# ChuhanZhou/News_Recommendation_Model

Hardware: NVIDIA B200
Metric: train_impressions_per_sec (higher is better)
Workload: dtype f32 (pair products as 3 x bf16 tcgen05 MMAs, fp32 accumulate; meets the fp32 tolerances)

## Files before the change

news_recommendation_model_b200/csrc/nrm_api.cu:

```cuda
#include <cstdarg>
#include <cstdio>
#include <cstring>
#include <mutex>
#include <vector>

#include "nrm_kernels.cuh"

namespace nrm {

static thread_local char g_err[512] = "";

void set_error(const char* fmt, ...) {
  va_list ap;
  va_start(ap, fmt);
  vsnprintf(g_err, sizeof(g_err), fmt, ap);
  va_end(ap);
}
int cuda_fail(cudaError_t e, const char* what) {
  set_error("CUDA error %d (%s) at %s", (int)e, cudaGetErrorString(e), what);
  return NRM_ECUDA;
}
int current_device() {
  int dev = 0;
  if (cudaGetDevice(&dev) != cudaSuccess || dev < 0 || dev >= 64) return 0;
// ... 22 lines not shown

KernelTimer::KernelTimer(const char* name, cudaStream_t stream) : slot_(-1), stream_(stream) {
  if (!g_timing) return;
  std::lock_guard<std::mutex> lock(g_timer_mu);
  int s = -1;
  for (int i = 0; i < g_ntimers; ++i) if (strcmp(g_timers[i].name, name) == 0) { s = i; break; }
  if (s < 0) { if (g_ntimers == kTimerSlots) return; s = g_ntimers++; g_timers[s].name = name; g_timers[s].used = 0; g_timers[s].made = false; }
  TimerSlot& t = g_timers[s];
  if (!t.made) { for (int i = 0; i < kTimerRing; ++i) { cudaEventCreate(&t.beg[i]); cudaEventCreate(&t.end[i]); } t.made = true; }
  if (t.used >= kTimerRing) return;
  slot_ = s;
  cudaEventRecord(t.beg[t.used], stream_);
}
KernelTimer::~KernelTimer() {
  if (slot_ < 0) return;
  std::lock_guard<std::mutex> lock(g_timer_mu);
  TimerSlot& t = g_timers[slot_];
  cudaEventRecord(t.end[t.used], stream_);
  t.used++;
}

struct SideStream {
  int dev; cudaStream_t caller;
  cudaStream_t stream; cudaEvent_t fork, join, fork2, join2, fork0, join0, join_tp, fork3, join3, fork4, join4;
  bool head_wgrad_pending = false; const float* wg_params = nullptr; float* wg_grads = nullptr; int wg_tiles = 0, wg_precision = 0;
};
static std::mutex g_side_mu;
static std::vector<SideStream*> g_sides;
static SideStream* side_stream(cudaStream_t caller) {
  const int dev = current_device();
  std::lock_guard<std::mutex> lock(g_side_mu);
  for (SideStream* p : g_sides)
    if (p->dev == dev && p->caller == caller) return p;
  SideStream* ss = new SideStream();
  ss->dev = dev; ss->caller = caller;
  bool ok = cudaStreamCreateWithFlags(&ss->stream, cudaStreamNonBlocking) == cudaSuccess;
  cudaEvent_t* evs[] = {&ss->fork, &ss->join, &ss->fork2, &ss->join2, &ss->fork0, &ss->join0, &ss->join_tp, &ss->fork3, &ss->join3,
                        &ss->fork4, &ss->join4};
  for (cudaEvent_t* e : evs) ok = ok && cudaEventCreateWithFlags(e, cudaEventDisableTiming) == cudaSuccess;
  if (!ok) { delete ss; return nullptr; }
  g_sides.push_back(ss);
  return ss;
}

bool use_rowstacked() {
  static const bool on = getenv("NRM_ATT_ITEM_TILES") == nullptr;
  return on;
}

bool w1_forward_on_tensor_cores(const Workspace&) {
  static const bool on = getenv("NRM_W1_FWD_TC") != nullptr;
  return on;
}

bool pdl_enabled() {
  static const bool on = getenv("NRM_NO_PDL") == nullptr;
  return on;
}

struct LayoutEntry { const char* name; long long offset; long long numel; };
// ... 44 lines not shown
  w.B = B; w.H = H; w.C = C;
  w.NH = (long long)B * H; w.R = (long long)B * C; w.N = w.NH + w.R;
  size_t off = 0;
  auto take = [&](size_t bytes) -> void* {
    void* p = base ? (char*)base + off : nullptr;
    off += (bytes + 255) & ~(size_t)255;
    return p;
  };
  const size_t f = sizeof(float);
  const size_t NH = (size_t)w.NH, R = (size_t)w.R, N = (size_t)w.N;
  w.xin_h = (float*)take(f * NH * XIN);
  w.xh = (float*)take(f * NH * 64);
  w.pca_h = (float*)take(f * NH * 64);
  w.e = (float*)take(f * R * E);
  w.mean = (float*)take(f * E);
  w.rstd = (float*)take(f * E);
  w.bn_sums = (double*)take(sizeof(double) * 2 * E);
  w.stat_part = (double*)take(sizeof(double) * STAT_BLOCKS * 2 * E);
  w.a1 = (float*)take(f * R * HID);
  w.gate = (float*)take(f * R * E);
  w.a2 = (float*)take(f * R * HID);
  w.y = (float*)take(f * R * E);
  w.a3 = (float*)take(f * R * HID);
  w.head_wt = (float*)take(f * (HEAD_WT_W1T + 64 * XIN));
  w.att_derived = (float*)take(f * 2 * 12420);
  w.tp = (float*)take(f * 2 * R * 64);
  w.att_rs_img = (float*)take(attention_rs_image_bytes());
  w.head_img = (float*)take(head_tc_image_bytes());
  w.head_arrive = (unsigned int*)take(256);
  if (training) {
    w.da3 = (float*)take(f * R * HID); w.da2 = (float*)take(f * R * HID); w.da1 = (float*)take(f * R * HID);
    w.dy = (float*)take(f * R * E);
    w.dgate = (float*)take(f * R * E);
    w.de = (float*)take(f * R * E);
    w.dz = (float*)take(f * R * E);
    w.bn_bwd_sums = (double*)take(sizeof(double) * 2 * E);
    w.head_part_f = (float*)take(f * ((R + 31) / 32) * 68);
    w.head_part_bn = (double*)take(sizeof(double) * ((R + 31) / 32) * 2 * E);
    w.head_part_w = (float*)take(f * 5 * HEAD_WG_CHUNKS_MAX * (HID * E + E));
    w.dxh = (float*)take(f * NH * 64);
    w.dxt = (float*)take(f * R * 64);
    w.dxin_h = (float*)take(f * NH * XIN);
    {
      const size_t ffma = (size_t)ATT_BWD_CTAS_MAX * ATT_PARTIAL, tc = (size_t)ATT_TC_PARTS_MAX * ATT_TC_PARTIAL;
      w.att_part = (float*)take(f * 2 * (ffma > tc ? ffma : tc));
    }
    w.dtp = (float*)take(f * 2 * R * 64);
// ... 29 lines not shown
  if (B <= 0 || H <= 0 || C <= 0) { set_error("%s: B, H, C must be positive (got %d, %d, %d)", fn, B, H, C); return NRM_EINVAL; }
  if (((long long)B * H + (long long)B * C) * 6 >= (1LL << 31)) { set_error("%s: batch too large for 32-bit entry ids", fn); return NRM_EINVAL; }
  return NRM_OK;
}
static int get_workspace(const char* fn, Workspace& w, void* ws, size_t ws_bytes, int B, int H, int C, int mode) {
  if (ws == nullptr || ((uintptr_t)ws & 255) != 0) { set_error("%s: workspace must be non-null and 256-byte aligned", fn); return NRM_EWORKSPACE; }
  const size_t need = carve_workspace(w, ws, B, H, C, mode);
  if (need > ws_bytes) { set_error("%s: workspace too small (%zu < %zu bytes)", fn, ws_bytes, need); return NRM_EWORKSPACE; }
  return NRM_OK;
}

static int encoder_forward(const BatchPtrs& in, const float* P, Workspace& w, int mode, int precision, cudaStream_t s) {
  SideStream* ss = side_stream(s);
  if (ss == nullptr) { set_error("encoder_forward: cannot create the side stream"); return NRM_ECUDA; }
  const bool tc = precision != NRM_PRECISION_FP32;
  NRM_CUDA(cudaEventRecord(ss->fork0, s));
  NRM_CUDA(cudaStreamWaitEvent(ss->stream, ss->fork0, 0));
  NRM_TRY(launch_head_transpose(P, w, ss->stream));
  NRM_CUDA(cudaEventRecord(ss->join0, ss->stream));
  if (tc) {
    if (use_rowstacked()) NRM_TRY(launch_attention_prep_rs(P, w, ss->stream)); else NRM_TRY(launch_attention_prep(P, w, ss->stream));
    if (head_on_tensor_cores(precision)) NRM_TRY(launch_head_images_tc(P, w, precision, (mode & NRM_MODE_KEEP_FOR_BWD) != 0, ss->stream));
  }
  { KernelTimer t("embed_rows", s);
    NRM_TRY(launch_embed_rows(in, P, w, (mode & NRM_MODE_KEEP_FOR_BWD) != 0, s)); }
  NRM_CUDA(cudaEventRecord(ss->fork, s));
  NRM_CUDA(cudaStreamWaitEvent(ss->stream, ss->fork, 0));
  if (tc) NRM_TRY(launch_candidate_tp(P, w, ss->stream));
  NRM_CUDA(cudaEventRecord(ss->join_tp, ss->stream));
  if (mode & NRM_MODE_KEEP_FOR_BWD) {
    NRM_TRY(launch_table_sort(w, ss->stream));
    NRM_CUDA(cudaEventRecord(ss->join, ss->stream));
  }
  NRM_CUDA(cudaStreamWaitEvent(s, ss->join0, 0));
  { KernelTimer t("w1_forward", s);
    if (tc && use_rowstacked() && w1_forward_on_tensor_cores(w)) NRM_TRY(launch_w1_forward_tc(P, w, precision, s)); else NRM_TRY(launch_w1_forward(P, w, s)); }
  NRM_CUDA(cudaStreamWaitEvent(s, ss->join_tp, 0));
  if (!tc) {
    { KernelTimer t("attention_forward_label", s); NRM_TRY(launch_attention_forward(in, P, w, 0, precision, s)); }
    { KernelTimer t("attention_forward_textimg", s); NRM_TRY(launch_attention_forward(in, P, w, 1, precision, s)); }
  } else {
    KernelTimer t("attention_forward", s);
    if (use_rowstacked()) {
      NRM_TRY(launch_attention_forward_rs(in, w, precision, s));
    } else {
      NRM_TRY(launch_attention_forward(in, P, w, 0, precision, s));
      NRM_TRY(launch_attention_forward(in, P, w, 1, precision, s));
    }
  }
  if (mode & NRM_MODE_KEEP_FOR_BWD) NRM_CUDA(cudaStreamWaitEvent(s, ss->join, 0));
  return NRM_OK;
}

static int encoder_backward(const BatchPtrs& in, const float* P, Workspace& w, int precision, float* G, cudaStream_t s) {
  SideStream* ss = side_stream(s);
  if (ss == nullptr) { set_error("encoder_backward: cannot create the side stream"); return NRM_ECUDA; }
  { KernelTimer t("attention_backward_label", s); NRM_TRY(launch_attention_backward(in, P, w, 0, precision, s)); }
  if (precision != NRM_PRECISION_FP32 && use_rowstacked()) {
    KernelTimer t("attention_input_grad_label", s);
    NRM_TRY(launch_attention_input_grad_rs(w, precision, s));
// ... 47 lines not shown
      NRM_CUDA(cudaEventSynchronize(t.end[k]));
      NRM_CUDA(cudaEventElapsedTime(&ms, t.beg[k], t.end[k]));
      total += ms;
    }
    float t_beg = 0.f, t_end = 0.f;
    if (t.used > 0 && g_ntimers > 0 && g_timers[0].used > 0) {
      cudaEventElapsedTime(&t_beg, g_timers[0].beg[g_timers[0].used - 1], t.beg[t.used - 1]);
      cudaEventElapsedTime(&t_end, g_timers[0].beg[g_timers[0].used - 1], t.end[t.used - 1]);
    }
    const int n = snprintf(buf + off, buf_bytes - off, "%s %d %.6f %.6f %.6f\n", t.name, t.used, total, t_beg, t_end);
    if (n < 0 || (size_t)n >= buf_bytes - off) break;
    off += (size_t)n;
  }
  return NRM_OK;
}
extern "C" int nrm_debug_rsprof(long long* host_out64) { return rsprof_read(host_out64); }
extern "C" long long nrm_debug_ws_field(int B, int H, int C, int mode, const char* name, long long* bytes) {
  if (B <= 0 || H <= 0 || C <= 0 || !name || !bytes) return -1;
  Workspace w;
  carve_workspace(w, reinterpret_cast<void*>(uintptr_t(256)), B, H, C, mode);
  const size_t R = (size_t)w.R, NH = (size_t)w.NH;
  struct F { const char* n; const void* p; size_t b; };
  const F fields[] = {{"e", w.e, R * E * 4}, {"de", w.de, R * E * 4}, {"dz", w.dz, R * E * 4}, {"dxh", w.dxh, NH * 64 * 4}, {"dxt", w.dxt, R * 64 * 4},
                      {"dxin_h", w.dxin_h, NH * XIN * 4}, {"att_dhid", w.att_dhid, (size_t)attention_rs_tiles(B, H, C) * 2 * 16384},
                      {"att_sc", w.att_sc, (size_t)attention_rs_tiles(B, H, C) * 512 * 4}, {"xh", w.xh, NH * 64 * 4}, {"dtp", w.dtp, 2 * R * 64 * 4},
                      {"tp", w.tp, 2 * R * 64 * 4}};
  for (const F& f : fields)
    if (strcmp(f.n, name) == 0 && f.p != nullptr) { *bytes = (long long)f.b; return (long long)(reinterpret_cast<uintptr_t>(f.p) - 256); }
  return -1;
}
extern "C" int nrm_debug_headprof(long long* host_out32) { return headprof_read(host_out32); }
extern "C" const char* nrm_last_error(void) { return g_err; }
extern "C" int nrm_layout_entries(void) { return kLayoutEntries; }
extern "C" const char* nrm_layout_name(int i) { return (i >= 0 && i < kLayoutEntries) ? kLayout[i].name : nullptr; }
extern "C" long long nrm_layout_offset(int i) { return (i >= 0 && i < kLayoutEntries) ? kLayout[i].offset : -1; }
extern "C" long long nrm_layout_numel(int i) { return (i >= 0 && i < kLayoutEntries) ? kLayout[i].numel : -1; }
extern "C" long long nrm_layout_fixed_floats(void) { return P_DELTA; }

extern "C" size_t nrm_workspace_bytes(int B, int H, int C, int mode) {
  if (B <= 0 || H <= 0 || C <= 0) return 0;
  Workspace w;
  return carve_workspace(w, nullptr, B, H, C, mode);
}

extern "C" size_t nrm_workspace_e_offset(int B, int H, int C, int mode) {
  if (B <= 0 || H <= 0 || C <= 0) return 0;
  Workspace w;
// ... 314 lines not shown
```

news_recommendation_model_b200/csrc/nrm_attention_tc.cu:

```cuda
#include "nrm_kernels.cuh"
#include <cstddef>

#include "nrm_umma.cuh"

namespace nrm {

#ifdef NRM_TC_PROFILE
__device__ long long g_tcprof[32];
#define TCPROF_DECL long long tcp_t = clock64();
#define TCPROF(i) do { if (blockIdx.x == 0 && (threadIdx.x == 0 || threadIdx.x == 32)) { const long long n__ = clock64(); g_tcprof[(i) + (threadIdx.x ? 16 : 0)] += n__ - tcp_t; tcp_t = n__; } } while (0)
#else
#define TCPROF_DECL
#define TCPROF(i) do { } while (0)
#endif

constexpr int TC_THREADS = 256;
constexpr int TC_MAXC = 8;

constexpr int DER_WD = 0, DER_A = 4096, DER_W2 = 8192, DER_B2 = 8256, DER_SIZE = 12420;
__host__ __device__ constexpr int wda_index(int j, int k) { return (((k >> 3) * 2 + ((k >> 2) & 1)) * 64 + j) * 4 + (k & 3); }

__global__ void __launch_bounds__(256)
att_prep_kernel(const float* __restrict__ P, float* __restrict__ der) {
  pdl_wait();
  pdl_trigger();
  const AttOffsets off = blockIdx.y == 0 ? ATT_LABEL : ATT_TI;
  float* d = der + (long long)blockIdx.y * DER_SIZE;
  const float* W = P + off.fc1_w;
  for (int i = blockIdx.x * 256 + threadIdx.x; i < 4096; i += gridDim.x * 256) {
    const int j = i >> 6, k = i & 63;
    const float wa = W[j * 256 + k], wc = W[j * 256 + 128 + k], wd = W[j * 256 + 192 + k];
    d[DER_WD + wda_index(j, k)] = wd;
    d[DER_A + wda_index(j, k)] = wa - wc;
  }
  if (blockIdx.x == 0 && threadIdx.x < 64) {
    d[DER_W2 + threadIdx.x] = P[off.fc2_w + threadIdx.x];
    if (threadIdx.x == 0) d[DER_B2] = P[off.fc2_b];
  }
}

__global__ void __launch_bounds__(256)
candidate_tp_kernel(const float* __restrict__ P, const float* __restrict__ e, long long R, float* __restrict__ tp_all) {
  pdl_wait();
  pdl_trigger();
  __shared__ float st[32][65];
  __shared__ float sBT[64][65];
  const AttOffsets off = blockIdx.y == 0 ? ATT_LABEL : ATT_TI;
  const int toff = blockIdx.y == 0 ? E_XT : E_PCAT;
  const float* W = P + off.fc1_w;
  float* tp = tp_all + (long long)blockIdx.y * R * 64;
  const int tid = threadIdx.x;
  const long long r0 = (long long)blockIdx.x * 32;
  const int nr = (int)min(32LL, R - r0);
  for (int i = tid; i < 32 * 64; i += 256) {
    const int r = i >> 6, k = i & 63;
    st[r][k] = r < nr ? __ldg(e + (r0 + r) * E + toff + k) : 0.f;
  }
  for (int i = tid; i < 64 * 64; i += 256) {
    const int j = i >> 6, k = i & 63;
    sBT[k][j] = __ldg(W + j * 256 + 64 + k) + __ldg(W + j * 256 + 128 + k);
  }
  __syncthreads();
  const int r = tid >> 3, jq = tid & 7;
  float v[8];
#pragma unroll
  for (int i = 0; i < 8; ++i) v[i] = __ldg(P + off.fc1_b + jq + 8 * i);
#pragma unroll 4
  for (int k = 0; k < 64; ++k) {
    const float tv = st[r][k];
#pragma unroll
    for (int i = 0; i < 8; ++i) v[i] = fmaf(sBT[k][jq + 8 * i], tv, v[i]);
  }
  if (r < nr) {
#pragma unroll
    for (int i = 0; i < 8; ++i) tp[(r0 + r) * 64 + jq + 8 * i] = v[i];
  }
}

constexpr uint32_t T8_LBO = 128, T8_SBO = 128, T8_BYTES = 1024;
__device__ __forceinline__ umma::Operand op_tile8_k(uint32_t addr) { return umma::make_operand(addr, T8_LBO, T8_SBO, 2 * T8_LBO, T8_BYTES); }
constexpr uint32_t T16_LBO = 256;
__device__ __forceinline__ umma::Operand op_tile16_k(uint32_t addr) { return umma::make_operand(addr, T16_LBO, 128, 2 * T16_LBO, 2 * T8_BYTES); }

template <int NP> struct TileBytes { static constexpr uint32_t T64 = NP * umma::TILE64_BYTES, T8 = NP * T8_BYTES; };

__device__ __forceinline__ void stage_item(int it, int& row, int& kb) {
  const int lane = it & 31, w = it >> 5;
  row = (w & 3) * 16 + (lane & 15);
  kb = (w >> 2) * 2 + (lane >> 4);
}
template <int BRANCH, int NP>
__device__ __forceinline__ void stage_history(const double* __restrict__ xh, const float* __restrict__ xhp,
                                              long long b, int H, int r0, unsigned char* tile) {
  constexpr int ITERS = 64 * 8 / TC_THREADS;
  if (BRANCH == 0) {
    float4 raw[ITERS][2];
#pragma unroll
    for (int u = 0; u < ITERS; ++u) {
// ... 899 lines not shown
      else umma::mma_product<SPLIT, 4>(d, umma::op_tile64_k(aa), umma::op_tile64_mn(bb), umma::make_idesc_bf16(64, 64, false, true), false);
    }
    umma::mma_commit(mbar);
  }
  umma::mbar_wait(mbar, 0);
  umma::fence_after_sync();
  const int half = lane >> 4, row = (warp & 3) * 16 + (lane & 15), cb = warp >> 2;
  {
    float v[32];
    umma::tmem_ld32(tmem + ((uint32_t)((warp & 3) * 32) << 16) + cb * 32, v);
#pragma unroll
    for (int j = 0; j < 32; ++j) out[(half * 64 + row) * 64 + cb * 32 + j] = v[j];
  }
  umma::fence_before_sync();
  __syncthreads();
  if (warp == 0) umma::tmem_dealloc(tmem, 64);
}

int launch_attention_prep(const float* P, Workspace& w, cudaStream_t s) {
  launch_pdl(att_prep_kernel, dim3(dim3(4, 2)), dim3(256), 0, s, P, w.att_derived);
  NRM_LAUNCH_CHECK("att_prep_kernel");
  return NRM_OK;
}
int launch_candidate_tp(const float* P, Workspace& w, cudaStream_t s) {
  launch_pdl(candidate_tp_kernel, dim3(dim3((unsigned)((w.R + 31) / 32), 2)), dim3(256), 0, s, P, w.e, w.R, w.tp);
  NRM_LAUNCH_CHECK("candidate_tp_kernel");
  return NRM_OK;
}

static size_t padded_smem(size_t need, int per_sm) {
  const size_t floor_bytes = (227 * 1024) / (per_sm + 1) + 1024;
  return need > floor_bytes ? need : floor_bytes;
}

template <int SPLIT>
static int launch_fwd_both(const BatchPtrs& in, Workspace& w, cudaStream_t s) {
  constexpr int NP = SPLIT == 3 ? 2 : 1;
  const int per_sm = 2;
  const size_t smem = padded_smem(sizeof(TcSmemFwd<NP>), per_sm);
  if (smem > 227 * 1024) { set_error("attention forward: shared memory"); return NRM_EUNSUPPORTED; }
  const long long npairs = (w.B + 1) / 2, units = npairs * w.C;
  const int grid = (int)min(max(npairs, (units + TC_MAXC - 1) / TC_MAXC), (long long)per_sm * sm_count());
  NRM_CUDA(cudaFuncSetAttribute(attention_forward_tc_kernel<SPLIT>, cudaFuncAttributeMaxDynamicSharedMemorySize, (int)smem));
  launch_pdl(attention_forward_tc_kernel<SPLIT>, dim3(dim3(grid, 2)), dim3(TC_THREADS), smem, s, in.xh, w.xh, w.B, w.H, w.C, w.att_derived, w.tp, w.e);
  NRM_LAUNCH_CHECK("attention_forward_tc_kernel");
  return NRM_OK;
}

int launch_attention_forward_tc(const BatchPtrs& in, Workspace& w, int branch, int precision, cudaStream_t s) {
  if (branch != 0) return NRM_OK;
  return precision == NRM_PRECISION_BF16 ? launch_fwd_both<1>(in, w, s) : launch_fwd_both<3>(in, w, s);
// ... 170 lines not shown
```

news_recommendation_model_b200/csrc/nrm_common.cuh:

```cuda
#pragma once
#include <cuda_runtime.h>
#include <stdint.h>
#include <stddef.h>
#include <math.h>

#include "../../include/nrm_b200.h"

namespace nrm {

constexpr int D = 64;
constexpr int HC = 80;
constexpr int TC = 78;
constexpr int GC = 3;
constexpr int XIN = 66;
constexpr int E = 264;
constexpr int HID = 66;
constexpr int NCAT = 3000, NTYPE = 16, NYEAR = 100, NMONTH = 13, NDAY = 32, NHOUR = 24;
constexpr int NKEY32 = NCAT;
constexpr int K8_TYPE = 0, K8_YEAR = 16, K8_MONTH = 116, K8_DAY = 129, K8_HOUR = 161;
constexpr int NKEY8 = 185;
constexpr float BN_EPS = 1e-5f;
constexpr float BN_MOMENTUM = 0.1f;

constexpr int E_LAB = 0, E_TI = 64, E_INST = 128, E_XT = 136, E_PCAT = 200;
// ... 86 lines not shown
  bool first_time() {
    const int d = current_device();
    if (__atomic_load_n(&done[d], __ATOMIC_ACQUIRE)) return false;
    __atomic_store_n(&done[d], (unsigned char)1, __ATOMIC_RELEASE);
    return true;
  }
};

struct KernelTimer {
  KernelTimer(const char* name, cudaStream_t stream);
  ~KernelTimer();
  int slot_; cudaStream_t stream_;
};

constexpr int SORT_CHUNK = 2048;
constexpr int SEG_GROUP = 128;
constexpr int ATT_BWD_CTAS_MAX = 148;
constexpr int ATT_PARTIAL = 3 * D * D + 64 + 64 + 4;
constexpr int ATT_TC_PARTS_MAX = 512;
constexpr int ATT_TC_PARTIAL = 2 * 4096 + 68;
constexpr int HEAD_WG_CHUNKS_MAX = 64;
constexpr int STAT_BLOCKS = 256;
constexpr int HEAD_WT_W1T = 5 * HID * E;
constexpr int W1_SPLITS = 256;

struct Workspace {
  int B, H, C;
  long long NH, R, N;
  float* xin_h;
  float* xh;
  float* pca_h;
  float* e;
  float* mean;
  float* rstd;
  double* bn_sums;
  double* stat_part;
  float* a1;
  float* gate;
  float* a2;
  float* y;
  float* a3;
  float* head_wt;
  float* head_part_f;
  double* head_part_bn;
  float* head_part_w;
  float* att_derived;
// ... 93 lines not shown
```

news_recommendation_model_b200/csrc/nrm_head_fused.cu:

```cuda
#include "nrm_kernels.cuh"
#include "nrm_umma.cuh"

namespace nrm {

constexpr int HT_ROWS = 36;
constexpr int HT_RPT = 9;
constexpr int HT_CONSUMERS = 288;
constexpr int HT_THREADS = 320;
constexpr int LDW = 268;
constexpr int LDN = 68;

constexpr int WCHUNK = 64 * HID;
constexpr int W_STAGES = 3;
constexpr int W_LAYER_CHUNKS = 5;
constexpr int W_CHUNKS = 5 * W_LAYER_CHUNKS;
struct HeadSmem {
  __align__(16) float w0[HT_ROWS * LDW];
  __align__(16) float w1[HT_ROWS * LDW];
  __align__(16) float nb[HT_ROWS * LDN];
  __align__(16) float wbuf[W_STAGES][WCHUNK];
  uint64_t full[W_STAGES];
  uint64_t empty[W_STAGES];
};

constexpr int WT_G1 = 0, WT_G2 = HID * E, WT_M1 = 2 * HID * E, WT_M2 = 3 * HID * E, WT_O1 = 4 * HID * E, WT_TOTAL = 5 * HID * E;
static_assert(WT_TOTAL == HEAD_WT_W1T, "w1^T follows the five head matrices in the transposed-weights buffer");

__global__ void __launch_bounds__(256)
head_transpose_kernel(const float* __restrict__ P, float* __restrict__ wt) {
  pdl_wait();
  pdl_trigger();
  const int m = blockIdx.y;
  const long long src_off[6] = {P_GATE_FC1_W, P_GATE_FC2_W, P_MLP_FC1_W, P_MLP_FC2_W, P_OUT_FC1_W, P_W1_W};
  const int rows = m == 5 ? 64 : (m == 1 || m == 3) ? E : HID;
  const int cols = m == 5 ? XIN : (m == 1 || m == 3) ? HID : E;
  const float* src = P + src_off[m];
  float* dst = wt + (long long)m * HID * E;
  for (int i = blockIdx.x * 256 + threadIdx.x; i < rows * cols; i += gridDim.x * 256) {
    const int c = i / rows, r = i - c * rows;
    dst[i] = __ldg(src + r * cols + c);
  }
}

struct HeadLayerDesc { const float* W; int K; int nout; };

__device__ __forceinline__ void consumer_sync() { __syncwarp(); asm volatile("bar.sync 1, %0;\n" ::"n"(HT_CONSUMERS) : "memory"); }

__device__ __forceinline__ void weight_producer(HeadSmem& sm, const HeadLayerDesc (&layers)[5]) {
  for (int g = 0; g < W_CHUNKS; ++g) {
    const int l = g / W_LAYER_CHUNKS, c = g - l * W_LAYER_CHUNKS;
    const int kc = WCHUNK / layers[l].nout;
    const int rows = min(kc, layers[l].K - c * kc);
    const float* src = layers[l].W + (long long)c * kc * layers[l].nout;
    const uint32_t bytes = (uint32_t)(rows * layers[l].nout * sizeof(float));
    const int slot = g % W_STAGES, use = g / W_STAGES;
// ... 538 lines not shown
        const int nb = (layer == 1 || layer == 3) ? E : HID;
        if (bi < nb) grads[b_off[layer] + bi] = v;
      }
    } else {
      if (i < HID) grads[P_OUT_FC2_W + i] = v; else grads[P_OUT_FC2_B] = v;
    }
  } else {
    const double v = ((red[0][lane] + red[1][lane]) + red[2][lane]) + red[3][lane];
    bn_bwd_sums[i] = v;
    if (i < E) grads[P_BN_B + i] = (float)v; else grads[P_BN_W + (i - E)] = (float)v;
  }
}

static inline int head_tiles(long long R) { return (int)((R + HT_ROWS - 1) / HT_ROWS); }
int head_wgrad_chunks(long long R) {
  int n = (2 * sm_count() + 4) / 5;
  const int maxn = (int)((R + WG_TILE - 1) / WG_TILE);
  if (n > maxn) n = maxn;
  if (n > HEAD_WG_CHUNKS_MAX) n = HEAD_WG_CHUNKS_MAX;
  return n < 1 ? 1 : n;
}

int launch_head_transpose(const float* P, Workspace& w, cudaStream_t s) {
  launch_pdl(head_transpose_kernel, dim3(dim3(8, 6)), dim3(256), 0, s, P, w.head_wt);
  NRM_LAUNCH_CHECK("head_transpose_kernel");
  return NRM_OK;
}

int launch_head_forward_fused(const float* P, Workspace& w, float* run_mean, float* run_var, long long* nbt, int training, int keep,
                              const double* bn_sums, long long bn_rows, float* logits, cudaStream_t s) {
  static DeviceOnce configured;
  if (configured.first_time()) {
    NRM_CUDA(cudaFuncSetAttribute(head_forward_kernel, cudaFuncAttributeMaxDynamicSharedMemorySize, (int)sizeof(HeadSmem)));
    NRM_CUDA(cudaFuncSetAttribute(head_backward_kernel, cudaFuncAttributeMaxDynamicSharedMemorySize, (int)sizeof(HeadSmem)));
  }
  launch_pdl(head_forward_kernel, dim3(head_tiles(w.R)), dim3(HT_THREADS), sizeof(HeadSmem), s, w.e, bn_sums, bn_rows, training, run_mean, run_var, nbt, w.mean, w.rstd, P, w.head_wt, w.R, keep, w.a1, w.gate, w.a2, w.y, w.a3, logits);
  NRM_LAUNCH_CHECK("head_forward_kernel");
  return NRM_OK;
}

static void head_wgrad_shape(const Workspace& w, int& rpc, int& nchunks) {
  const int nch = head_wgrad_chunks(w.R);
  rpc = (int)((w.R + nch - 1) / nch);
  rpc = (rpc + WG_TILE - 1) / WG_TILE * WG_TILE;
  nchunks = (int)((w.R + rpc - 1) / rpc);
}

// ... 47 lines not shown
```

news_recommendation_model_b200/csrc/nrm_kernels.cuh:

```cuda
#pragma once
#include "nrm_common.cuh"

namespace nrm {

struct CompactPtrs {
  const float* articles; int n_articles;
  const int* hist_article; const unsigned* hist_time; const float* hist_click;
  const int* cand_article; const unsigned* cand_time;
  const float* label32; double* label64;
};
struct BatchPtrs {
  const double* xh;
  const double* xt; long long xt_bs;
  const double* xg; long long xg_bs;
  const CompactPtrs* compact = nullptr;
};

int launch_embed_rows(const BatchPtrs& in, const float* P, Workspace& w, bool with_keys, cudaStream_t s);
int launch_table_sort(Workspace& w, cudaStream_t s);
int launch_table_grads(Workspace& w, float* grads, cudaStream_t s);
int launch_small_linear_grads(const BatchPtrs& in, Workspace& w, float* grads, cudaStream_t s);

int launch_w1_forward(const float* P, Workspace& w, cudaStream_t s);
int launch_w1_backward(const float* P, Workspace& w, float* grads, cudaStream_t s);

int launch_w1_forward_tc(const float* P, Workspace& w, int precision, cudaStream_t s);
int launch_w1_backward_tc(const float* P, Workspace& w, float* grads, int precision, cudaStream_t s);

int launch_attention_forward(const BatchPtrs& in, const float* P, Workspace& w, int branch, int precision, cudaStream_t s);
int launch_attention_backward(const BatchPtrs& in, const float* P, Workspace& w, int branch, int precision, cudaStream_t s);
int launch_attention_finish(const float* P, Workspace& w, int branch, int precision, float* grads, cudaStream_t s);

int launch_attention_prep(const float* P, Workspace& w, cudaStream_t s);
int launch_candidate_tp(const float* P, Workspace& w, cudaStream_t s);
int launch_attention_forward_tc(const BatchPtrs& in, Workspace& w, int branch, int precision, cudaStream_t s);
int launch_attention_backward_tc(const BatchPtrs& in, const float* P, Workspace& w, int branch, int precision, cudaStream_t s);
int launch_attention_finish_tc(const float* P, Workspace& w, float* grads, cudaStream_t s);

size_t attention_rs_image_bytes();
int rsprof_read(long long* host_out64);
int launch_attention_prep_rs(const float* P, Workspace& w, cudaStream_t s);
int launch_attention_forward_rs(const BatchPtrs& in, Workspace& w, int precision, cudaStream_t s);
int launch_attention_forward_rs_scores(Workspace& w, int precision, cudaStream_t s);
int launch_attention_backward_rs(Workspace& w, int branch, int precision, bool export_dhid, cudaStream_t s);
int launch_attention_input_grad_rs(Workspace& w, int precision, cudaStream_t s);
long long attention_rs_tiles(int B, int H, int C);
bool use_rowstacked();

int launch_head_transpose(const float* P, Workspace& w, cudaStream_t s);
int launch_head_forward_fused(const float* P, Workspace& w, float* run_mean, float* run_var, long long* nbt, int training, int keep,
                              const double* bn_sums, long long bn_rows, float* logits, cudaStream_t s);
int launch_head_backward_dgrad(const float* P, Workspace& w, const float* dlogits, cudaStream_t s);
int launch_head_backward_bn(Workspace& w, float* grads, cudaStream_t s, int dgrad_tiles);
int launch_head_backward_wgrad(const float* P, Workspace& w, float* grads, cudaStream_t s, int dgrad_tiles, int tc_precision = 0);
int launch_head_backward_fused(const float* P, Workspace& w, const float* dlogits, float* grads, cudaStream_t s);

size_t head_tc_image_bytes();
// ... 24 lines not shown
```

news_recommendation_model_b200/csrc/nrm_w1.cu:

```cuda
#include "nrm_kernels.cuh"

namespace nrm {

constexpr int W1_ROWS = 128, W1_THREADS = 256;
constexpr int W1F_ROWS = 64, W1F_THREADS = 128;
constexpr int W1_PART = 64 * XIN + 64;

template <int THREADS = W1_THREADS>
__device__ __forceinline__ void copy_tile(float* dst, const float* __restrict__ src, int nfloats) {
  const int n4 = nfloats >> 2;
  for (int i = threadIdx.x; i < n4; i += THREADS) {
    const unsigned d = (unsigned)__cvta_generic_to_shared(dst + 4 * i);
    asm volatile("cp.async.cg.shared.global [%0], [%1], 16;\n" ::"r"(d), "l"(src + 4 * i) : "memory");
  }
  for (int i = (n4 << 2) + threadIdx.x; i < nfloats; i += THREADS) dst[i] = __ldg(src + i);
}
__device__ __forceinline__ void copy_wait() { asm volatile("cp.async.wait_all;\n" ::: "memory"); }

struct W1SmemFwd { __align__(16) float xs[W1F_ROWS * XIN]; __align__(16) float wt[XIN * 64]; };

__global__ void __launch_bounds__(W1F_THREADS, 6)
w1_forward_kernel(const float* __restrict__ xin, const float* __restrict__ P, const float* __restrict__ w1t, float* __restrict__ xh,
                  long long NH) {
  pdl_wait();
  pdl_trigger();
  extern __shared__ __align__(16) unsigned char w1_raw[];
  W1SmemFwd& sm = *reinterpret_cast<W1SmemFwd*>(w1_raw);
  const int tid = threadIdx.x, rg = tid >> 4, cg = tid & 15;
  const long long ntiles = (NH + W1F_ROWS - 1) / W1F_ROWS;
  long long tile = blockIdx.x;
  if (tile < ntiles) copy_tile<W1F_THREADS>(sm.xs, xin + tile * W1F_ROWS * XIN, (int)min((long long)W1F_ROWS, NH - tile * W1F_ROWS) * XIN);
  copy_tile<W1F_THREADS>(sm.wt, w1t, XIN * 64);
  const float4 bias = __ldg(reinterpret_cast<const float4*>(P + P_W1_B) + cg);
  for (; tile < ntiles; tile += gridDim.x) {
    const long long r0 = tile * W1F_ROWS;
    const int nr = (int)min((long long)W1F_ROWS, NH - r0);
    copy_wait();
    __syncthreads();
    float acc[8][4];
#pragma unroll
    for (int i = 0; i < 8; ++i) { acc[i][0] = bias.x; acc[i][1] = bias.y; acc[i][2] = bias.z; acc[i][3] = bias.w; }
    const float* xr = sm.xs + rg * 8 * XIN;
#pragma unroll 2
    for (int k = 0; k < XIN; ++k) {
      const float4 w = *reinterpret_cast<const float4*>(sm.wt + k * 64 + 4 * cg);
#pragma unroll
      for (int i = 0; i < 8; ++i) {
        const float a = xr[i * XIN + k];
        acc[i][0] = fmaf(a, w.x, acc[i][0]); acc[i][1] = fmaf(a, w.y, acc[i][1]);
        acc[i][2] = fmaf(a, w.z, acc[i][2]); acc[i][3] = fmaf(a, w.w, acc[i][3]);
      }
    }
    __syncthreads();
    const long long nt = tile + gridDim.x;
    if (nt < ntiles) copy_tile<W1F_THREADS>(sm.xs, xin + nt * W1F_ROWS * XIN, (int)min((long long)W1F_ROWS, NH - nt * W1F_ROWS) * XIN);
#pragma unroll
    for (int i = 0; i < 8; ++i)
      if (rg * 8 + i < nr)
        *reinterpret_cast<float4*>(xh + (r0 + rg * 8 + i) * 64 + 4 * cg) = make_float4(acc[i][0], acc[i][1], acc[i][2], acc[i][3]);
  }
}

struct W1SmemBwd { __align__(16) float ds[W1_ROWS * 64]; __align__(16) float xs[W1_ROWS * XIN]; __align__(16) float w[64 * XIN]; };

__global__ void __launch_bounds__(W1_THREADS, 2)
w1_backward_kernel(const float* __restrict__ xin, const float* __restrict__ dxh, const float* __restrict__ P,
                   float* __restrict__ dxin, long long NH, float* __restrict__ part) {
  pdl_wait();
  pdl_trigger();
  extern __shared__ __align__(16) unsigned char w1_raw[];
  W1SmemBwd& sm = *reinterpret_cast<W1SmemBwd*>(w1_raw);
  const int tid = threadIdx.x, rg = tid >> 4, cg = tid & 15;
  for (int i = tid; i < 64 * XIN; i += W1_THREADS) sm.w[i] = __ldg(P + P_W1_W + i);
  float dw[4][5];
#pragma unroll
  for (int a = 0; a < 4; ++a)
#pragma unroll
    for (int t = 0; t < 5; ++t) dw[a][t] = 0.f;
  float db[4] = {0.f, 0.f, 0.f, 0.f};
  const int c4 = min(cg + 64, XIN - 1);
  const long long ntiles = (NH + W1_ROWS - 1) / W1_ROWS;
  for (long long tile = blockIdx.x; tile < ntiles; tile += gridDim.x) {
// ... 63 lines not shown
    for (int t = 0; t < 4; ++t) out[(4 * rg + a) * XIN + cg + 16 * t] = dw[a][t];
    if (cg + 64 < XIN) out[(4 * rg + a) * XIN + cg + 64] = dw[a][4];
    if (cg == 0) out[64 * XIN + 4 * rg + a] = db[a];
  }
}

__global__ void __launch_bounds__(256)
w1_finish_kernel(const float* __restrict__ part, int nparts, float* __restrict__ grads) {
  pdl_wait();
  pdl_trigger();
  __shared__ float red[4][64];
  const int lane = threadIdx.x & 63, grp = threadIdx.x >> 6;
  const int i = blockIdx.x * 64 + lane;
  float s = 0.f;
  if (i < W1_PART)
    for (int p = grp; p < nparts; p += 4) s += part[(long long)p * W1_PART + i];
  red[grp][lane] = s;
  __syncthreads();
  if (grp == 0 && i < W1_PART) grads[P_W1_W + i] = ((red[0][lane] + red[1][lane]) + red[2][lane]) + red[3][lane];
}

static_assert(P_W1_B == P_W1_W + 64 * XIN, "w1.weight / w1.bias must be contiguous in the flat layout");

int launch_w1_forward(const float* P, Workspace& w, cudaStream_t s) {
  static DeviceOnce configured;
  if (configured.first_time()) {
    NRM_CUDA(cudaFuncSetAttribute(w1_forward_kernel, cudaFuncAttributeMaxDynamicSharedMemorySize, (int)sizeof(W1SmemFwd)));
    NRM_CUDA(cudaFuncSetAttribute(w1_backward_kernel, cudaFuncAttributeMaxDynamicSharedMemorySize, (int)sizeof(W1SmemBwd)));
  }
  const long long ntiles = (w.NH + W1F_ROWS - 1) / W1F_ROWS;
  const int grid = (int)min(ntiles, (long long)6 * sm_count());
  launch_pdl(w1_forward_kernel, dim3(grid), dim3(W1F_THREADS), sizeof(W1SmemFwd), s, w.xin_h, P, w.head_wt + HEAD_WT_W1T, w.xh, w.NH);
  NRM_LAUNCH_CHECK("w1_forward_kernel");
  return NRM_OK;
}

int launch_w1_finish(Workspace& w, int nparts, float* G, cudaStream_t s) {
  launch_pdl(w1_finish_kernel, dim3((W1_PART + 63) / 64), dim3(256), 0, s, w.splitk, nparts, G);
  NRM_LAUNCH_CHECK("w1_finish_kernel");
  return NRM_OK;
}

int launch_w1_backward(const float* P, Workspace& w, float* G, cudaStream_t s) {
  static DeviceOnce configured;
  if (configured.first_time()) {
    NRM_CUDA(cudaFuncSetAttribute(w1_backward_kernel, cudaFuncAttributeMaxDynamicSharedMemorySize, (int)sizeof(W1SmemBwd)));
  }
  const long long ntiles = (w.NH + W1_ROWS - 1) / W1_ROWS;
  const int grid = (int)min(ntiles, (long long)min(2 * sm_count(), W1_SPLITS));
  launch_pdl(w1_backward_kernel, dim3(grid), dim3(W1_THREADS), sizeof(W1SmemBwd), s, w.xin_h, w.dxh, P, w.dxin_h, w.NH, w.splitk);
  NRM_LAUNCH_CHECK("w1_backward_kernel");
  launch_pdl(w1_finish_kernel, dim3((W1_PART + 63) / 64), dim3(256), 0, s, w.splitk, grid, G);
  NRM_LAUNCH_CHECK("w1_finish_kernel");
  return NRM_OK;
}
// ... 3 lines not shown
```

Measured before the change: 1.816 million.

## Fold candidate tp projection into the w1 forward kernel as extra tiles

Removes the separate candidate_tp kernel on the side stream and instead appends candidate-projection tiles (two per row block, one per attention branch) to the persistent w1_forward tile loop. The summed fc1 weight slices are precomputed once by extra blocks of the head transpose kernel into a new workspace region. This cuts one launch and the fork/join it needed, and reuses the w1 kernel's tiled FMA and cp.async pipeline. In exchange the tp work now runs on the main stream, serialized after embed_rows instead of overlapping with it, and the weight tile in shared memory must be reloaded whenever a block switches tile type.

```diff
diff --git a/news_recommendation_model_b200/csrc/nrm_api.cu b/news_recommendation_model_b200/csrc/nrm_api.cu
--- a/news_recommendation_model_b200/csrc/nrm_api.cu
+++ b/news_recommendation_model_b200/csrc/nrm_api.cu
@@ -68,7 +68,7 @@
 
 struct SideStream {
   int dev; cudaStream_t caller;
-  cudaStream_t stream; cudaEvent_t fork, join, fork2, join2, fork0, join0, join_tp, fork3, join3, fork4, join4;
+  cudaStream_t stream; cudaEvent_t fork, join, fork2, join2, fork0, join0, join_prep, fork3, join3, fork4, join4;
   bool head_wgrad_pending = false; const float* wg_params = nullptr; float* wg_grads = nullptr; int wg_tiles = 0, wg_precision = 0;
 };
 static std::mutex g_side_mu;
@@ -81,7 +81,7 @@
   SideStream* ss = new SideStream();
   ss->dev = dev; ss->caller = caller;
   bool ok = cudaStreamCreateWithFlags(&ss->stream, cudaStreamNonBlocking) == cudaSuccess;
-  cudaEvent_t* evs[] = {&ss->fork, &ss->join, &ss->fork2, &ss->join2, &ss->fork0, &ss->join0, &ss->join_tp, &ss->fork3, &ss->join3,
+  cudaEvent_t* evs[] = {&ss->fork, &ss->join, &ss->fork2, &ss->join2, &ss->fork0, &ss->join0, &ss->join_prep, &ss->fork3, &ss->join3,
                         &ss->fork4, &ss->join4};
   for (cudaEvent_t* e : evs) ok = ok && cudaEventCreateWithFlags(e, cudaEventDisableTiming) == cudaSuccess;
   if (!ok) { delete ss; return nullptr; }
@@ -172,7 +172,7 @@
   w.a2 = (float*)take(f * R * HID);
   w.y = (float*)take(f * R * E);
   w.a3 = (float*)take(f * R * HID);
-  w.head_wt = (float*)take(f * (HEAD_WT_W1T + 64 * XIN));
+  w.head_wt = (float*)take(f * HEAD_WT_SIZE);
   w.att_derived = (float*)take(f * 2 * 12420);
   w.tp = (float*)take(f * 2 * R * 64);
   w.att_rs_img = (float*)take(attention_rs_image_bytes());
@@ -248,20 +248,24 @@
     if (use_rowstacked()) NRM_TRY(launch_attention_prep_rs(P, w, ss->stream)); else NRM_TRY(launch_attention_prep(P, w, ss->stream));
     if (head_on_tensor_cores(precision)) NRM_TRY(launch_head_images_tc(P, w, precision, (mode & NRM_MODE_KEEP_FOR_BWD) != 0, ss->stream));
   }
+  NRM_CUDA(cudaEventRecord(ss->join_prep, ss->stream));
   { KernelTimer t("embed_rows", s);
     NRM_TRY(launch_embed_rows(in, P, w, (mode & NRM_MODE_KEEP_FOR_BWD) != 0, s)); }
-  NRM_CUDA(cudaEventRecord(ss->fork, s));
-  NRM_CUDA(cudaStreamWaitEvent(ss->stream, ss->fork, 0));
-  if (tc) NRM_TRY(launch_candidate_tp(P, w, ss->stream));
-  NRM_CUDA(cudaEventRecord(ss->join_tp, ss->stream));
   if (mode & NRM_MODE_KEEP_FOR_BWD) {
+    NRM_CUDA(cudaEventRecord(ss->fork, s));
+    NRM_CUDA(cudaStreamWaitEvent(ss->stream, ss->fork, 0));
     NRM_TRY(launch_table_sort(w, ss->stream));
     NRM_CUDA(cudaEventRecord(ss->join, ss->stream));
   }
   NRM_CUDA(cudaStreamWaitEvent(s, ss->join0, 0));
   { KernelTimer t("w1_forward", s);
-    if (tc && use_rowstacked() && w1_forward_on_tensor_cores(w)) NRM_TRY(launch_w1_forward_tc(P, w, precision, s)); else NRM_TRY(launch_w1_forward(P, w, s)); }
-  NRM_CUDA(cudaStreamWaitEvent(s, ss->join_tp, 0));
+    if (tc && use_rowstacked() && w1_forward_on_tensor_cores(w)) {
+      NRM_TRY(launch_w1_forward_tc(P, w, precision, s));
+      NRM_TRY(launch_w1_forward(P, w, false, true, s));
+    } else {
+      NRM_TRY(launch_w1_forward(P, w, true, tc, s));
+    } }
+  NRM_CUDA(cudaStreamWaitEvent(s, ss->join_prep, 0));
   if (!tc) {
     { KernelTimer t("attention_forward_label", s); NRM_TRY(launch_attention_forward(in, P, w, 0, precision, s)); }
     { KernelTimer t("attention_forward_textimg", s); NRM_TRY(launch_attention_forward(in, P, w, 1, precision, s)); }
@@ -355,7 +359,7 @@
   const size_t R = (size_t)w.R, NH = (size_t)w.NH;
   struct F { const char* n; const void* p; size_t b; };
   const F fields[] = {{"e", w.e, R * E * 4}, {"de", w.de, R * E * 4}, {"dz", w.dz, R * E * 4}, {"dxh", w.dxh, NH * 64 * 4}, {"dxt", w.dxt, R * 64 * 4},
-                      {"dxin_h", w.dxin_h, NH * XIN * 4}, {"att_dhid", w.att_dhid, (size_t)attention_rs_tiles(B, H, C) * 2 * 16384},
+                      {"dxin_h", w.dxin_h, NH * XIN * 4}, {"xin_h", w.xin_h, NH * XIN * 4}, {"att_dhid", w.att_dhid, (size_t)attention_rs_tiles(B, H, C) * 2 * 16384},
                       {"att_sc", w.att_sc, (size_t)attention_rs_tiles(B, H, C) * 512 * 4}, {"xh", w.xh, NH * 64 * 4}, {"dtp", w.dtp, 2 * R * 64 * 4},
                       {"tp", w.tp, 2 * R * 64 * 4}};
   for (const F& f : fields)
diff --git a/news_recommendation_model_b200/csrc/nrm_attention_tc.cu b/news_recommendation_model_b200/csrc/nrm_attention_tc.cu
--- a/news_recommendation_model_b200/csrc/nrm_attention_tc.cu
+++ b/news_recommendation_model_b200/csrc/nrm_attention_tc.cu
@@ -36,44 +36,6 @@
   if (blockIdx.x == 0 && threadIdx.x < 64) {
     d[DER_W2 + threadIdx.x] = P[off.fc2_w + threadIdx.x];
     if (threadIdx.x == 0) d[DER_B2] = P[off.fc2_b];
-  }
-}
-
-__global__ void __launch_bounds__(256)
-candidate_tp_kernel(const float* __restrict__ P, const float* __restrict__ e, long long R, float* __restrict__ tp_all) {
-  pdl_wait();
-  pdl_trigger();
-  __shared__ float st[32][65];
-  __shared__ float sBT[64][65];
-  const AttOffsets off = blockIdx.y == 0 ? ATT_LABEL : ATT_TI;
-  const int toff = blockIdx.y == 0 ? E_XT : E_PCAT;
-  const float* W = P + off.fc1_w;
-  float* tp = tp_all + (long long)blockIdx.y * R * 64;
-  const int tid = threadIdx.x;
-  const long long r0 = (long long)blockIdx.x * 32;
-  const int nr = (int)min(32LL, R - r0);
-  for (int i = tid; i < 32 * 64; i += 256) {
-    const int r = i >> 6, k = i & 63;
-    st[r][k] = r < nr ? __ldg(e + (r0 + r) * E + toff + k) : 0.f;
-  }
-  for (int i = tid; i < 64 * 64; i += 256) {
-    const int j = i >> 6, k = i & 63;
-    sBT[k][j] = __ldg(W + j * 256 + 64 + k) + __ldg(W + j * 256 + 128 + k);
-  }
-  __syncthreads();
-  const int r = tid >> 3, jq = tid & 7;
-  float v[8];
-#pragma unroll
-  for (int i = 0; i < 8; ++i) v[i] = __ldg(P + off.fc1_b + jq + 8 * i);
-#pragma unroll 4
-  for (int k = 0; k < 64; ++k) {
-    const float tv = st[r][k];
-#pragma unroll
-    for (int i = 0; i < 8; ++i) v[i] = fmaf(sBT[k][jq + 8 * i], tv, v[i]);
-  }
-  if (r < nr) {
-#pragma unroll
-    for (int i = 0; i < 8; ++i) tp[(r0 + r) * 64 + jq + 8 * i] = v[i];
   }
 }
 
@@ -1019,11 +981,6 @@
   NRM_LAUNCH_CHECK("att_prep_kernel");
   return NRM_OK;
 }
-int launch_candidate_tp(const float* P, Workspace& w, cudaStream_t s) {
-  launch_pdl(candidate_tp_kernel, dim3(dim3((unsigned)((w.R + 31) / 32), 2)), dim3(256), 0, s, P, w.e, w.R, w.tp);
-  NRM_LAUNCH_CHECK("candidate_tp_kernel");
-  return NRM_OK;
-}
 
 static size_t padded_smem(size_t need, int per_sm) {
   const size_t floor_bytes = (227 * 1024) / (per_sm + 1) + 1024;
diff --git a/news_recommendation_model_b200/csrc/nrm_common.cuh b/news_recommendation_model_b200/csrc/nrm_common.cuh
--- a/news_recommendation_model_b200/csrc/nrm_common.cuh
+++ b/news_recommendation_model_b200/csrc/nrm_common.cuh
@@ -132,6 +132,8 @@
 constexpr int HEAD_WG_CHUNKS_MAX = 64;
 constexpr int STAT_BLOCKS = 256;
 constexpr int HEAD_WT_W1T = 5 * HID * E;
+constexpr int HEAD_WT_TPW = HEAD_WT_W1T + 64 * XIN;
+constexpr int HEAD_WT_SIZE = HEAD_WT_TPW + 2 * 64 * 64;
 constexpr int W1_SPLITS = 256;
 
 struct Workspace {
diff --git a/news_recommendation_model_b200/csrc/nrm_head_fused.cu b/news_recommendation_model_b200/csrc/nrm_head_fused.cu
--- a/news_recommendation_model_b200/csrc/nrm_head_fused.cu
+++ b/news_recommendation_model_b200/csrc/nrm_head_fused.cu
@@ -31,6 +31,15 @@
   pdl_wait();
   pdl_trigger();
   const int m = blockIdx.y;
+  if (m >= 6) {
+    const float* W = P + (m == 6 ? P_LA_FC1_W : P_TI_FC1_W);
+    float* dst = wt + HEAD_WT_TPW + (m - 6) * 4096;
+    for (int i = blockIdx.x * 256 + threadIdx.x; i < 4096; i += gridDim.x * 256) {
+      const int k = i >> 6, j = i & 63;
+      dst[i] = __ldg(W + j * 256 + 64 + k) + __ldg(W + j * 256 + 128 + k);
+    }
+    return;
+  }
   const long long src_off[6] = {P_GATE_FC1_W, P_GATE_FC2_W, P_MLP_FC1_W, P_MLP_FC2_W, P_OUT_FC1_W, P_W1_W};
   const int rows = m == 5 ? 64 : (m == 1 || m == 3) ? E : HID;
   const int cols = m == 5 ? XIN : (m == 1 || m == 3) ? HID : E;
@@ -615,7 +624,7 @@
 }
 
 int launch_head_transpose(const float* P, Workspace& w, cudaStream_t s) {
-  launch_pdl(head_transpose_kernel, dim3(dim3(8, 6)), dim3(256), 0, s, P, w.head_wt);
+  launch_pdl(head_transpose_kernel, dim3(dim3(8, 8)), dim3(256), 0, s, P, w.head_wt);
   NRM_LAUNCH_CHECK("head_transpose_kernel");
   return NRM_OK;
 }
diff --git a/news_recommendation_model_b200/csrc/nrm_kernels.cuh b/news_recommendation_model_b200/csrc/nrm_kernels.cuh
--- a/news_recommendation_model_b200/csrc/nrm_kernels.cuh
+++ b/news_recommendation_model_b200/csrc/nrm_kernels.cuh
@@ -21,7 +21,7 @@
 int launch_table_grads(Workspace& w, float* grads, cudaStream_t s);
 int launch_small_linear_grads(const BatchPtrs& in, Workspace& w, float* grads, cudaStream_t s);
 
-int launch_w1_forward(const float* P, Workspace& w, cudaStream_t s);
+int launch_w1_forward(const float* P, Workspace& w, bool history, bool build_tp, cudaStream_t s);
 int launch_w1_backward(const float* P, Workspace& w, float* grads, cudaStream_t s);
 
 int launch_w1_forward_tc(const float* P, Workspace& w, int precision, cudaStream_t s);
@@ -32,7 +32,6 @@
 int launch_attention_finish(const float* P, Workspace& w, int branch, int precision, float* grads, cudaStream_t s);
 
 int launch_attention_prep(const float* P, Workspace& w, cudaStream_t s);
-int launch_candidate_tp(const float* P, Workspace& w, cudaStream_t s);
 int launch_attention_forward_tc(const BatchPtrs& in, Workspace& w, int branch, int precision, cudaStream_t s);
 int launch_attention_backward_tc(const BatchPtrs& in, const float* P, Workspace& w, int branch, int precision, cudaStream_t s);
 int launch_attention_finish_tc(const float* P, Workspace& w, float* grads, cudaStream_t s);
diff --git a/news_recommendation_model_b200/csrc/nrm_w1.cu b/news_recommendation_model_b200/csrc/nrm_w1.cu
--- a/news_recommendation_model_b200/csrc/nrm_w1.cu
+++ b/news_recommendation_model_b200/csrc/nrm_w1.cu
@@ -19,45 +19,72 @@
 
 struct W1SmemFwd { __align__(16) float xs[W1F_ROWS * XIN]; __align__(16) float wt[XIN * 64]; };
 
+template <int K, int LD>
+__device__ __forceinline__ void w1f_tile_product(const W1SmemFwd& sm, const float4 bias, float (&acc)[8][4]) {
+  const int rg = threadIdx.x >> 4, cg = threadIdx.x & 15;
+#pragma unroll
+  for (int i = 0; i < 8; ++i) { acc[i][0] = bias.x; acc[i][1] = bias.y; acc[i][2] = bias.z; acc[i][3] = bias.w; }
+  const float* xr = sm.xs + rg * 8 * LD;
+#pragma unroll 2
+  for (int k = 0; k < K; ++k) {
+    const float4 w = *reinterpret_cast<const float4*>(sm.wt + k * 64 + 4 * cg);
+#pragma unroll
+    for (int i = 0; i < 8; ++i) {
+      const float a = xr[i * LD + k];
+      acc[i][0] = fmaf(a, w.x, acc[i][0]); acc[i][1] = fmaf(a, w.y, acc[i][1]);
+      acc[i][2] = fmaf(a, w.z, acc[i][2]); acc[i][3] = fmaf(a, w.w, acc[i][3]);
+    }
+  }
+}
+
+__device__ __forceinline__ void w1f_issue_tile(W1SmemFwd& sm, long long tile, long long nh, const float* __restrict__ xin, long long NH,
+                                               const float* __restrict__ wt, const float* __restrict__ e, long long R) {
+  if (tile < nh) {
+    copy_tile<W1F_THREADS>(sm.xs, xin + tile * W1F_ROWS * XIN, (int)min((long long)W1F_ROWS, NH - tile * W1F_ROWS) * XIN);
+    return;
+  }
+  const long long u = tile - nh, r0 = (u >> 1) * W1F_ROWS;
+  const int branch = (int)(u & 1), nr = (int)min((long long)W1F_ROWS, R - r0);
+  copy_tile<W1F_THREADS>(sm.wt, wt + HEAD_WT_TPW + branch * 4096, 4096);
+  const float* src = e + r0 * E + (branch == 0 ? E_XT : E_PCAT);
+  for (int i = threadIdx.x; i < nr * 16; i += W1F_THREADS) {
+    const unsigned d = (unsigned)__cvta_generic_to_shared(sm.xs + (i >> 4) * 64 + (i & 15) * 4);
+    asm volatile("cp.async.cg.shared.global [%0], [%1], 16;\n" ::"r"(d), "l"(src + (long long)(i >> 4) * E + (i & 15) * 4) : "memory");
+  }
+}
+
 __global__ void __launch_bounds__(W1F_THREADS, 6)
-w1_forward_kernel(const float* __restrict__ xin, const float* __restrict__ P, const float* __restrict__ w1t, float* __restrict__ xh,
-                  long long NH) {
+w1_forward_kernel(const float* __restrict__ xin, const float* __restrict__ P, const float* __restrict__ wt, float* __restrict__ xh,
+                  long long NH, const float* __restrict__ e, long long R, float* __restrict__ tp) {
   pdl_wait();
   pdl_trigger();
   extern __shared__ __align__(16) unsigned char w1_raw[];
   W1SmemFwd& sm = *reinterpret_cast<W1SmemFwd*>(w1_raw);
   const int tid = threadIdx.x, rg = tid >> 4, cg = tid & 15;
-  const long long ntiles = (NH + W1F_ROWS - 1) / W1F_ROWS;
+  const long long nh = xh != nullptr ? (NH + W1F_ROWS - 1) / W1F_ROWS : 0;
+  const long long ntiles = nh + (tp != nullptr ? 2 * ((R + W1F_ROWS - 1) / W1F_ROWS) : 0);
   long long tile = blockIdx.x;
-  if (tile < ntiles) copy_tile<W1F_THREADS>(sm.xs, xin + tile * W1F_ROWS * XIN, (int)min((long long)W1F_ROWS, NH - tile * W1F_ROWS) * XIN);
-  copy_tile<W1F_THREADS>(sm.wt, w1t, XIN * 64);
-  const float4 bias = __ldg(reinterpret_cast<const float4*>(P + P_W1_B) + cg);
+  if (tile < nh) copy_tile<W1F_THREADS>(sm.wt, wt + HEAD_WT_W1T, XIN * 64);
+  if (tile < ntiles) w1f_issue_tile(sm, tile, nh, xin, NH, wt, e, R);
   for (; tile < ntiles; tile += gridDim.x) {
-    const long long r0 = tile * W1F_ROWS;
-    const int nr = (int)min((long long)W1F_ROWS, NH - r0);
+    const bool hist = tile < nh;
+    const float* bias = hist ? P + P_W1_B : P + (((tile - nh) & 1) == 0 ? P_LA_FC1_B : P_TI_FC1_B);
+    const float4 b = __ldg(reinterpret_cast<const float4*>(bias) + cg);
     copy_wait();
     __syncthreads();
     float acc[8][4];
-#pragma unroll
-    for (int i = 0; i < 8; ++i) { acc[i][0] = bias.x; acc[i][1] = bias.y; acc[i][2] = bias.z; acc[i][3] = bias.w; }
-    const float* xr = sm.xs + rg * 8 * XIN;
-#pragma unroll 2
-    for (int k = 0; k < XIN; ++k) {
-      const float4 w = *reinterpret_cast<const float4*>(sm.wt + k * 64 + 4 * cg);
-#pragma unroll
-      for (int i = 0; i < 8; ++i) {
-        const float a = xr[i * XIN + k];
-        acc[i][0] = fmaf(a, w.x, acc[i][0]); acc[i][1] = fmaf(a, w.y, acc[i][1]);
-        acc[i][2] = fmaf(a, w.z, acc[i][2]); acc[i][3] = fmaf(a, w.w, acc[i][3]);
-      }
-    }
+    if (hist) w1f_tile_product<XIN, XIN>(sm, b, acc); else w1f_tile_product<64, 64>(sm, b, acc);
     __syncthreads();
     const long long nt = tile + gridDim.x;
-    if (nt < ntiles) copy_tile<W1F_THREADS>(sm.xs, xin + nt * W1F_ROWS * XIN, (int)min((long long)W1F_ROWS, NH - nt * W1F_ROWS) * XIN);
+    if (nt < ntiles) w1f_issue_tile(sm, nt, nh, xin, NH, wt, e, R);
+    const long long u = tile - nh;
+    const long long r0 = hist ? tile * W1F_ROWS : (u >> 1) * W1F_ROWS;
+    const int nr = (int)min((long long)W1F_ROWS, (hist ? NH : R) - r0);
+    float* out = hist ? xh + r0 * 64 : tp + (u & 1) * R * 64 + r0 * 64;
 #pragma unroll
     for (int i = 0; i < 8; ++i)
       if (rg * 8 + i < nr)
-        *reinterpret_cast<float4*>(xh + (r0 + rg * 8 + i) * 64 + 4 * cg) = make_float4(acc[i][0], acc[i][1], acc[i][2], acc[i][3]);
+        *reinterpret_cast<float4*>(out + (long long)(rg * 8 + i) * 64 + 4 * cg) = make_float4(acc[i][0], acc[i][1], acc[i][2], acc[i][3]);
   }
 }
 
@@ -167,15 +194,17 @@
 
 static_assert(P_W1_B == P_W1_W + 64 * XIN, "w1.weight / w1.bias must be contiguous in the flat layout");
 
-int launch_w1_forward(const float* P, Workspace& w, cudaStream_t s) {
+int launch_w1_forward(const float* P, Workspace& w, bool history, bool build_tp, cudaStream_t s) {
   static DeviceOnce configured;
   if (configured.first_time()) {
     NRM_CUDA(cudaFuncSetAttribute(w1_forward_kernel, cudaFuncAttributeMaxDynamicSharedMemorySize, (int)sizeof(W1SmemFwd)));
     NRM_CUDA(cudaFuncSetAttribute(w1_backward_kernel, cudaFuncAttributeMaxDynamicSharedMemorySize, (int)sizeof(W1SmemBwd)));
   }
-  const long long ntiles = (w.NH + W1F_ROWS - 1) / W1F_ROWS;
+  const long long ntiles = (history ? (w.NH + W1F_ROWS - 1) / W1F_ROWS : 0) + (build_tp ? 2 * ((w.R + W1F_ROWS - 1) / W1F_ROWS) : 0);
+  if (ntiles == 0) return NRM_OK;
   const int grid = (int)min(ntiles, (long long)6 * sm_count());
-  launch_pdl(w1_forward_kernel, dim3(grid), dim3(W1F_THREADS), sizeof(W1SmemFwd), s, w.xin_h, P, w.head_wt + HEAD_WT_W1T, w.xh, w.NH);
+  launch_pdl(w1_forward_kernel, dim3(grid), dim3(W1F_THREADS), sizeof(W1SmemFwd), s, w.xin_h, P, w.head_wt, history ? w.xh : nullptr, w.NH,
+             w.e, w.R, build_tp ? w.tp : nullptr);
   NRM_LAUNCH_CHECK("w1_forward_kernel");
   return NRM_OK;
 }
```

After: 1.850 million (median of 6 runs). +1.8%, better.
